# unknownue/puflow

Measured on AMD Instinct MI355X. Metric: patches/sec x4 2048->8192 (PU1K discrete, eval), higher is better.
Workload: dtype f32 (split-fp16 MFMA products, fp32 accumulate); 1 GPU; BASELINE configs[1]: PU1K discrete x4 inference, 32 x 2048-pt patches per GPU (fp32-parity mode); patches_per_gpu=32, total_batch=32, npoint=2048

## Files before the change

### puflow_amd/csrc/knn.hip

```cpp
#include <hip/hip_runtime.h>
#include "pf_api_internal.h"
#include "pf_wave.h"
#include <type_traits>

#ifndef PF_KNN5
#define PF_KNN5 1
#endif
#ifndef PF_KNN5_NWMAX
#define PF_KNN5_NWMAX 16
#endif
#ifndef PF_KNN5_MIN_M
#define PF_KNN5_MIN_M 256
#endif
#ifndef PF_KNN5_MIN_WGS
#define PF_KNN5_MIN_WGS 64
#endif
typedef float f4 __attribute__((ext_vector_type(4)));

namespace {

__device__ __forceinline__ float sqdist(float qx, float qy, float qz, float rx, float ry, float rz) {
#pragma clang fp contract(off)
    const float dx = __fsub_rn(qx, rx), dy = __fsub_rn(qy, ry), dz = __fsub_rn(qz, rz);
    return __fadd_rn(__fadd_rn(__fmul_rn(dx, dx), __fmul_rn(dy, dy)), __fmul_rn(dz, dz));
}

__device__ __forceinline__ int knn_opaque(int v) { asm("" : "+v"(v)); return v; }

template <int K>
__device__ __forceinline__ void topk_insert(float (&bd)[K], int (&bi)[K], float d, int j) {
#pragma unroll
    for (int i = K - 1; i >= 1; --i) {
        const bool ltl = d < bd[i - 1], lti = d < bd[i];
        bi[i] = ltl ? knn_opaque(bi[i - 1]) : (lti ? j : knn_opaque(bi[i]));
        bd[i] = ltl ? bd[i - 1] : (lti ? d : bd[i]);
    }
    if (d < bd[0]) { bd[0] = d; bi[0] = j; }
}

template <int K, int T>
__device__ __forceinline__ void topk_insert_head(float (&bd)[K], int (&bi)[K], float d, int j) {
    constexpr int TOP = T < K - 1 ? T : K - 1;
#pragma unroll
    for (int i = TOP; i >= 1; --i) {
        const bool ltl = d < bd[i - 1], lti = d < bd[i];
        bi[i] = ltl ? knn_opaque(bi[i - 1]) : (lti ? j : knn_opaque(bi[i]));
        bd[i] = ltl ? bd[i - 1] : (lti ? d : bd[i]);
    }
    if (d < bd[0]) { bd[0] = d; bi[0] = j; }
}

template <int I, int N, class F>
__device__ __forceinline__ void pf_static_for_knn(F&& f) {
    if constexpr (I < N) {
        f(std::integral_constant<int, I>{});
        pf_static_for_knn<I + 1, N>(f);
    }
}

template <int K>
__device__ __forceinline__ void exact_scan(float qx, float qy, float qz, const float* __restrict__ r, int M,
                                           float (&bd)[K], int (&bi)[K]) {
#pragma unroll
    for (int i = 0; i < K; ++i) { bd[i] = __builtin_inff(); bi[i] = -1; }
    for (int j = 0; j < M; ++j) {
        const float d = sqdist(qx, qy, qz, r[j * 3 + 0], r[j * 3 + 1], r[j * 3 + 2]);
        if (d < bd[K - 1]) topk_insert<K>(bd, bi, d, j);
    }
}

template <int K>
__device__ __forceinline__ void store_topk(const float (&bd)[K], const int (&bi)[K], size_t row, int* __restrict__ idx_out,
                                           float* __restrict__ dist_out) {
    if (idx_out) {
        int* o = idx_out + row * K;
#pragma unroll
        for (int i = 0; i < K; ++i) o[i] = bi[i];
    }
    if (dist_out) {
        float* od = dist_out + row * K;
#pragma unroll
        for (int i = 0; i < K; ++i) od[i] = bd[i];
    }
}

template <int K>
__global__ __launch_bounds__(64) void knn_kernel(const float* __restrict__ p1, const float* __restrict__ p2,
                                                 int N, int M, int* __restrict__ idx_out,
                                                 float* __restrict__ dist_out) {
    const int b = blockIdx.y;
    const int n = blockIdx.x * 64 + threadIdx.x;
    const bool live = n < N;
    const float* q = p1 + ((size_t)b * N + (live ? n : N - 1)) * 3;
    const float qx = q[0], qy = q[1], qz = q[2];
    float bd[K];
    int bi[K];
    exact_scan<K>(qx, qy, qz, p2 + (size_t)b * M * 3, M, bd, bi);
    if (live) store_topk<K>(bd, bi, (size_t)b * N + n, idx_out, dist_out);
}

__device__ __forceinline__ void sort16(float (&v)[16]) {
#pragma unroll
    for (int k = 2; k <= 16; k <<= 1)
#pragma unroll
        for (int j = k >> 1; j > 0; j >>= 1)
#pragma unroll
            for (int i = 0; i < 16; ++i) {
                const int l = i ^ j;
                if (l > i) {
                    const float a = v[i], c = v[l];
                    const bool up = (i & k) == 0;
                    v[i] = up ? fminf(a, c) : fmaxf(a, c);
                    v[l] = up ? fmaxf(a, c) : fminf(a, c);
                }
            }
}

constexpr int KNN2_T = 256;
constexpr int KNN2_CAP = 64;

__device__ __forceinline__ float bcast(float v, int srclane) {
    return __builtin_bit_cast(float, __builtin_amdgcn_readlane(__builtin_bit_cast(int, v), srclane));
}

template <int K>
__global__ __launch_bounds__(KNN2_T) void knn2_kernel(const float* __restrict__ p1, const float* __restrict__ p2,
                                                      int N, int M, int* __restrict__ idx_out,
                                                      float* __restrict__ dist_out) {
    static_assert(K <= 16, "threshold selection uses two 16-element sorted halves");
    __shared__ unsigned short lst[KNN2_CAP][KNN2_T];
    const int b = blockIdx.y, tid = threadIdx.x, lane = tid & 63;
    const int n = blockIdx.x * KNN2_T + tid;
    const bool live = n < N;
    const float* q = p1 + ((size_t)b * N + (live ? n : N - 1)) * 3;
    const float qx = q[0], qy = q[1], qz = q[2];
    const float* __restrict__ r = p2 + (size_t)b * M * 3;

    auto load_ref = [&](int j0, float& cx, float& cy, float& cz) {
        const int j = j0 + lane;
        const bool in = j < M;
        const int jc = in ? j : M - 1;
        cx = in ? r[jc * 3 + 0] : __builtin_inff();
        cy = r[jc * 3 + 1];
        cz = r[jc * 3 + 2];
    };

    float gm[32];
#pragma unroll
    for (int g = 0; g < 32; ++g) gm[g] = __builtin_inff();
    {
        float cx, cy, cz;
        load_ref(0, cx, cy, cz);
        for (int j0 = 0; j0 < M; j0 += 64) {
            float nx = cx, ny = cy, nz = cz;
            if (j0 + 64 < M) load_ref(j0 + 64, nx, ny, nz);
#pragma unroll
            for (int c = 0; c < 64; ++c)
                gm[c & 31] = fminf(gm[c & 31], sqdist(qx, qy, qz, bcast(cx, c), bcast(cy, c), bcast(cz, c)));
            cx = nx; cy = ny; cz = nz;
        }
    }
    float tau;
    {
        float ha[16], hb[16];
#pragma unroll
        for (int g = 0; g < 16; ++g) { ha[g] = gm[g]; hb[g] = gm[16 + g]; }
        sort16(ha);
        sort16(hb);
        tau = fminf(ha[0], hb[K - 1]);
#pragma unroll
        for (int i = 1; i < K; ++i) tau = fmaxf(tau, fminf(ha[i], hb[K - 1 - i]));
    }

    int cnt = 0;
    {
        float cx, cy, cz;
        load_ref(0, cx, cy, cz);
        for (int j0 = 0; j0 < M; j0 += 64) {
            float nx = cx, ny = cy, nz = cz;
            if (j0 + 64 < M) load_ref(j0 + 64, nx, ny, nz);
#pragma unroll
            for (int c = 0; c < 64; ++c) {
                const float d = sqdist(qx, qy, qz, bcast(cx, c), bcast(cy, c), bcast(cz, c));
                if (d <= tau) {
                    if (cnt < KNN2_CAP) lst[cnt][tid] = (unsigned short)(j0 + c);
                    ++cnt;
                }
            }
            cx = nx; cy = ny; cz = nz;
        }
    }

    float bd[K];
    int bi[K];
    if (__any(cnt > KNN2_CAP)) {
        exact_scan<K>(qx, qy, qz, r, M, bd, bi);
    } else {
#pragma unroll
        for (int i = 0; i < K; ++i) { bd[i] = __builtin_inff(); bi[i] = -1; }
        for (int s = 0; __any(s < cnt); ++s) {
            if (s < cnt) {
                const int j = lst[s][tid];
                const float d = sqdist(qx, qy, qz, r[j * 3 + 0], r[j * 3 + 1], r[j * 3 + 2]);
                topk_insert<K>(bd, bi, d, j);
            }
        }
    }
    if (live) store_topk<K>(bd, bi, (size_t)b * N + n, idx_out, dist_out);
}

#ifndef PF_KNN4_U
#define PF_KNN4_U 32
#endif
constexpr int KNN4_U = PF_KNN4_U;

template <int K, int KNN4_W>
__global__ __launch_bounds__(KNN4_W * 64) void knn4_kernel(const float* __restrict__ p1, const float* __restrict__ p2,
                                                           int N, int M, int* __restrict__ idx_out,
                                                           float* __restrict__ dist_out) {
    static_assert(K <= 16, "threshold selection uses two 16-element sorted halves");
    constexpr int KNN4_G = 32 / KNN4_W;
    constexpr int KNN4_CAP = 32;
    __shared__ float gms[32][64];
    __shared__ unsigned short lst[KNN4_W][KNN4_CAP][64];
    __shared__ int cnts[KNN4_W][64];
    const int b = blockIdx.y, lane = threadIdx.x & 63;
    const int wave = __builtin_amdgcn_readfirstlane(threadIdx.x >> 6);
    const int n = blockIdx.x * 64 + lane;
    const bool live = n < N;
    const float* q = p1 + ((size_t)b * N + (live ? n : N - 1)) * 3;
    const float qx = q[0], qy = q[1], qz = q[2];
    const float* __restrict__ r = p2 + (size_t)b * M * 3;
    auto fdist = [&](int j) {
        const float* rr = r + (size_t)j * 3;
        const float dx = qx - rr[0], dy = qy - rr[1], dz = qz - rr[2];
        return fmaf(dz, dz, fmaf(dy, dy, dx * dx));
    };
    const int mq = ((M + KNN4_W * 64 - 1) / (KNN4_W * 64)) * 64;
    const int jb = wave * mq, je = min(jb + mq, M);
    const int jfull = jb + ((je - jb) > 0 ? ((je - jb) / KNN4_U) * KNN4_U : 0);

    {
        float gm[KNN4_G];
#pragma unroll
        for (int g = 0; g < KNN4_G; ++g) gm[g] = __builtin_inff();
        for (int j0 = jb; j0 < jfull; j0 += KNN4_U) {
#pragma unroll
            for (int c = 0; c < KNN4_U; ++c) gm[c % KNN4_G] = fminf(gm[c % KNN4_G], fdist(j0 + c));
        }
        for (int j0 = jfull; j0 < je; j0 += KNN4_G) {
#pragma unroll
            for (int g = 0; g < KNN4_G; ++g)
                if (j0 + g < je) gm[g] = fminf(gm[g], fdist(j0 + g));
        }
#pragma unroll
        for (int g = 0; g < KNN4_G; ++g) gms[wave * KNN4_G + g][lane] = gm[g];
    }
    __syncthreads();
    float tau;
    {
        float ha[16], hb[16];
#pragma unroll
        for (int g = 0; g < 16; ++g) { ha[g] = gms[g][lane]; hb[g] = gms[16 + g][lane]; }
        sort16(ha);
        sort16(hb);
        tau = fminf(ha[0], hb[K - 1]);
#pragma unroll
        for (int i = 1; i < K; ++i) tau = fmaxf(tau, fminf(ha[i], hb[K - 1 - i]));
        tau = fmaf(tau, 1.9073486328125e-6f, tau) + 1e-37f;
    }

#if defined(PF_KNN_ABL) && PF_KNN_ABL == 2
    if (wave == 0 && live) idx_out[((size_t)b * N + n) * K] = __float_as_int(tau);
    return;
#endif
    int cnt = 0;
    auto take = [&](float d, int j) {
        if (d <= tau) {
            if (cnt < KNN4_CAP) lst[wave][cnt][lane] = (unsigned short)j;
            ++cnt;
        }
    };
    for (int j0 = jb; j0 < jfull; j0 += KNN4_U) {
        float dd[KNN4_U];
#pragma unroll
        for (int c = 0; c < KNN4_U; ++c) dd[c] = fdist(j0 + c);
#pragma unroll
        for (int c = 0; c < KNN4_U; c += 4) {
            if (fminf(fminf(dd[c], dd[c + 1]), fminf(dd[c + 2], dd[c + 3])) <= tau) {
                take(dd[c], j0 + c); take(dd[c + 1], j0 + c + 1); take(dd[c + 2], j0 + c + 2); take(dd[c + 3], j0 + c + 3);
            }
        }
    }
    for (int j = jfull; j < je; ++j) take(fdist(j), j);
    cnts[wave][lane] = cnt;
#if defined(PF_KNN_ABL) && PF_KNN_ABL == 1
    __syncthreads();
    if (wave == 0 && live) idx_out[((size_t)b * N + n) * K] = cnt;
    return;
#endif
    if constexpr (KNN4_W == 4) {
        static_assert(KNN4_CAP * 2 >= K * 4, "a wave's list region is reused for its K sorted distances");
        __shared__ unsigned short sidx[4][K][64];
        float (*sdst)[64] = reinterpret_cast<float (*)[64]>(&lst[wave][0][0]);
        {
            float bd[K];
            int bi[K];
#pragma unroll
            for (int i = 0; i < K; ++i) { bd[i] = __builtin_inff(); bi[i] = 0xffff; }
            const int cme = cnt < KNN4_CAP ? cnt : KNN4_CAP;
            int j = cme > 0 ? (int)lst[wave][0][lane] : 0;
            float rx = r[j * 3 + 0], ry = r[j * 3 + 1], rz = r[j * 3 + 2];
            for (int t = 0; __any(t < cme); ++t) {
                const int jn = t + 1 < cme ? (int)lst[wave][t + 1][lane] : 0;
                const float nx = r[jn * 3 + 0], ny = r[jn * 3 + 1], nz = r[jn * 3 + 2];
                if (t < cme) topk_insert<K>(bd, bi, sqdist(qx, qy, qz, rx, ry, rz), j);
                j = jn; rx = nx; ry = ny; rz = nz;
            }
#pragma unroll
            for (int i = 0; i < K; ++i) { sdst[i][lane] = bd[i]; sidx[wave][i][lane] = (unsigned short)bi[i]; }
        }
        __syncthreads();
        if (wave != 0) return;
        float bd[K];
        int bi[K];
        if (__any(cnts[0][lane] > KNN4_CAP || cnts[1][lane] > KNN4_CAP || cnts[2][lane] > KNN4_CAP || cnts[3][lane] > KNN4_CAP)) {
            exact_scan<K>(qx, qy, qz, r, M, bd, bi);
        } else {
            float hd[4];
            int hi[4], hp[4];
#pragma unroll
            for (int w = 0; w < 4; ++w) {
                hd[w] = reinterpret_cast<const float (*)[64]>(&lst[w][0][0])[0][lane];
                hi[w] = sidx[w][0][lane];
                hp[w] = 1;
            }
#pragma unroll
            for (int i = 0; i < K; ++i) {
                int wm = 0;
                float dm = hd[0];
#pragma unroll
                for (int w = 1; w < 4; ++w)
                    if (hd[w] < dm) { dm = hd[w]; wm = w; }
                int im = hi[0];
#pragma unroll
                for (int w = 1; w < 4; ++w) im = wm == w ? hi[w] : im;
                bd[i] = dm; bi[i] = im;
                int pm = hp[0];
#pragma unroll
                for (int w = 1; w < 4; ++w) pm = wm == w ? hp[w] : pm;
                const int pc = pm < K ? pm : K - 1;
                const float nd = pm < K ? reinterpret_cast<const float (*)[64]>(&lst[wm][0][0])[pc][lane] : __builtin_inff();
                const int ni = sidx[wm][pc][lane];
#pragma unroll
                for (int w = 0; w < 4; ++w) {
                    const bool m = wm == w;
                    hd[w] = m ? nd : hd[w]; hi[w] = m ? ni : hi[w]; hp[w] = m ? pm + 1 : hp[w];
                }
            }
        }
        if (live) store_topk<K>(bd, bi, (size_t)b * N + n, idx_out, dist_out);
        return;
    }
    __syncthreads();
    bool over = false;
    int ctot = 0;
#pragma unroll
    for (int w = 0; w < KNN4_W; ++w) { over |= cnts[w][lane] > KNN4_CAP; ctot += cnts[w][lane]; }
    if (__any(over || ctot > 64)) {
        if (wave != 0) return;
        float bd[K];
        int bi[K];
        exact_scan<K>(qx, qy, qz, r, M, bd, bi);
        if (live) store_topk<K>(bd, bi, (size_t)b * N + n, idx_out, dist_out);
        return;
    }
    constexpr int QPW = 64 / KNN4_W;
    int jq[QPW], cq[QPW];
    float dq[QPW];
#pragma unroll
    for (int t = 0; t < QPW; ++t) {
        const int ql = wave * QPW + t;
        cq[t] = __builtin_amdgcn_readlane(ctot, ql);
        int j0 = 0x7fffffff, acc = 0;
#pragma unroll
        for (int w = 0; w < KNN4_W; ++w) {
            const int cw = cnts[w][ql];
            const int s0 = lane - acc;
            if (s0 >= 0 && s0 < cw) j0 = lst[w][s0][ql];
            acc += cw;
        }
        jq[t] = j0;
    }
#pragma unroll
    for (int t = 0; t < QPW; ++t) {
        const int ql = wave * QPW + t;
        const float ax = __builtin_bit_cast(float, __builtin_amdgcn_readlane(__builtin_bit_cast(int, qx), ql));
        const float ay = __builtin_bit_cast(float, __builtin_amdgcn_readlane(__builtin_bit_cast(int, qy), ql));
        const float az = __builtin_bit_cast(float, __builtin_amdgcn_readlane(__builtin_bit_cast(int, qz), ql));
        const int jj = lane < cq[t] ? jq[t] : 0;
        const float d = sqdist(ax, ay, az, r[(size_t)jj * 3 + 0], r[(size_t)jj * 3 + 1], r[(size_t)jj * 3 + 2]);
        dq[t] = lane < cq[t] ? d : __builtin_inff();
    }
#pragma unroll
    for (int t = 0; t < QPW; ++t) {
        const int ql = wave * QPW + t;
        const int nq = blockIdx.x * 64 + ql;
        if (nq >= N) break;
        const int C = cq[t];
        const float d0 = dq[t];
        const int j0 = jq[t];
        const size_t row = (size_t)b * N + nq;
        int r0 = 0;
        for (int c = 0; c < C; ++c) {
            const float dc = __builtin_bit_cast(float, __builtin_amdgcn_readlane(__builtin_bit_cast(int, d0), c));
            const int jc = __builtin_amdgcn_readlane(j0, c);
            r0 += (dc < d0 || (dc == d0 && jc < j0)) ? 1 : 0;
        }
        if (lane < C && r0 < K) { idx_out[row * K + r0] = j0; if (dist_out) dist_out[row * K + r0] = d0; }
    }
}

constexpr int KNN5_CAP = 32;
constexpr int KNN5_WB = 6144;
template <int K, int NW>
__global__ __launch_bounds__(NW * 64) void knn5_kernel(const float* __restrict__ p1, const float* __restrict__ p2, int N, int M,
                                                       int Mpad, int* __restrict__ idx_out, float* __restrict__ dist_out) {
    static_assert(K <= 16, "threshold selection uses two 16-element sorted halves");
    extern __shared__ float4 k5lds[];
    __shared__ float rmx[NW];
    const int b = blockIdx.y, lane = threadIdx.x & 63, wave = threadIdx.x >> 6;
    const int col = lane & 15, g = lane >> 4;
    const int n = (blockIdx.x * NW + wave) * 16 + col;
    const bool live = n < N;
    const float* __restrict__ r = p2 + (size_t)b * M * 3;
    float4* tab = k5lds;
    unsigned char* wsm = reinterpret_cast<unsigned char*>(k5lds + Mpad) + wave * KNN5_WB;
    float (*gms)[64] = reinterpret_cast<float (*)[64]>(wsm);
    unsigned short (*lst)[64] = reinterpret_cast<unsigned short (*)[64]>(wsm + 2048);
    float rm = 0.f;
    for (int j = threadIdx.x; j < Mpad; j += NW * 64) {
        float4 e = make_float4(0.f, 0.f, 0.f, __builtin_inff());
        if (j < M) {
            const float x = r[j * 3 + 0], y = r[j * 3 + 1], z = r[j * 3 + 2];
            const float R = fmaf(z, z, fmaf(y, y, x * x));
            e = make_float4(-2.f * x, -2.f * y, -2.f * z, R);
            rm = fmaxf(rm, R);
        }
        tab[j] = e;
    }
    rm = pf_xor_max<1, 32>(rm);
    if (lane == 0) rmx[wave] = rm;
    __syncthreads();
    float Rmax = rmx[0];
#pragma unroll
    for (int w = 1; w < NW; ++w) Rmax = fmaxf(Rmax, rmx[w]);
#if defined(PF_KNN_ABL) && PF_KNN_ABL == 3
    if (live && g == 0) idx_out[((size_t)b * N + n) * K] = __float_as_int(Rmax);
    return;
#endif
    if ((blockIdx.x * NW + wave) * 16 >= N) return;
    const float* qp = p1 + ((size_t)b * N + (live ? n : N - 1)) * 3;
    const float qx = qp[0], qy = qp[1], qz = qp[2];
    const float bq = g == 0 ? qx : (g == 1 ? qy : (g == 2 ? qz : 1.f));
    const float* tabf = reinterpret_cast<const float*>(tab) + col * 4 + g;
    const int nch = Mpad / 16;
    auto filtc = [&](int c, f4 acc) { return __builtin_amdgcn_mfma_f32_16x16x4f32(tabf[c * 64], bq, acc, 0, 0, 0); };
    auto filt = [&](int c) {
        const f4 z4 = {0.f, 0.f, 0.f, 0.f};
        return filtc(c, z4);
    };
    {
        float gm[8];
#pragma unroll
        for (int i = 0; i < 8; ++i) gm[i] = __builtin_inff();
        for (int c0 = 0; c0 < nch; c0 += 8) {
            f4 d[8];
#pragma unroll
            for (int u = 0; u < 8; ++u) d[u] = filt(c0 + u);
            __builtin_amdgcn_sched_barrier(0);
#pragma unroll
            for (int u = 0; u < 8; u += 4)
#pragma unroll
                for (int v = 0; v < 2; ++v)
#pragma unroll
                    for (int i = 0; i < 4; ++i)
                        gm[v * 4 + i] = __builtin_fminf(gm[v * 4 + i], __builtin_fminf(d[u + v][i], d[u + v + 2][i]));
        }
#pragma unroll
        for (int i = 0; i < 8; ++i) gms[i][lane] = gm[i];
    }
    __builtin_amdgcn_wave_barrier();
    float tau;
    {
        float ha[16], hb[16];
#pragma unroll
        for (int i = 0; i < 8; ++i) {
            ha[i] = gms[i][col]; ha[8 + i] = gms[i][col + 16];
            hb[i] = gms[i][col + 32]; hb[8 + i] = gms[i][col + 48];
        }
        if constexpr (K == 1) {
            tau = fminf(ha[0], hb[0]);
#pragma unroll
            for (int i = 1; i < 16; ++i) tau = fminf(tau, fminf(ha[i], hb[i]));
        } else {
            sort16(ha);
            sort16(hb);
            tau = fminf(ha[0], hb[K - 1]);
#pragma unroll
            for (int i = 1; i < K; ++i) tau = fmaxf(tau, fminf(ha[i], hb[K - 1 - i]));
        }
        const float s = __builtin_sqrtf(Rmax) + __builtin_sqrtf(fmaf(qz, qz, fmaf(qy, qy, qx * qx)));
        tau = fmaf(3.814697265625e-6f, s * s, tau) + 4e-37f;
    }
#if defined(PF_KNN_ABL) && PF_KNN_ABL == 2
    if (live && g == 0) idx_out[((size_t)b * N + n) * K] = __float_as_int(tau);
    return;
#endif
    int cnt = 0;
    const f4 ntau = {-tau, -tau, -tau, -tau};
    for (int c0 = 0; c0 < nch; c0 += 8) {
        f4 d[8];
#pragma unroll
        for (int u = 0; u < 8; ++u) d[u] = filtc(c0 + u, ntau);
        __builtin_amdgcn_sched_barrier(0);
        unsigned m0 = 0, m1 = 0, m2 = 0, m3 = 0;
#pragma unroll
        for (int s = 0; s < 8; ++s) {
            const int u = s >> 2, i = s & 3;
            asm("v_alignbit_b32 %0, %0, %4, 31\n\tv_alignbit_b32 %1, %1, %5, 31\n\t"
                "v_alignbit_b32 %2, %2, %6, 31\n\tv_alignbit_b32 %3, %3, %7, 31"
                : "+v"(m0), "+v"(m1), "+v"(m2), "+v"(m3)
                : "v"(d[u][i]), "v"(d[2 + u][i]), "v"(d[4 + u][i]), "v"(d[6 + u][i]));
        }
        unsigned mask = (m0 << 24) | (m1 << 16) | (m2 << 8) | m3;
        auto pop = [&]() {
            if (mask != 0) {
                const int p = __clz((int)mask);
                mask &= ~(0x80000000u >> p);
                lst[cnt & (KNN5_CAP - 1)][lane] = (unsigned short)((c0 + (p >> 2)) * 16 + 4 * g + (p & 3));
                ++cnt;
            }
        };
#if defined(PF_KNN_ABL) && PF_KNN_ABL == 6
        cnt += __popc(mask);
#else
        pop();
        pop();
        while (__any(mask != 0)) pop();
#endif
    }
#if defined(PF_KNN_ABL) && (PF_KNN_ABL == 1 || PF_KNN_ABL == 6)
    if (live && g == 0) idx_out[((size_t)b * N + n) * K] = cnt;
    return;
#endif
    float bd[K];
    int bi[K];
    {
#pragma unroll
        for (int i = 0; i < K; ++i) { bd[i] = __builtin_inff(); bi[i] = 0xffff; }
        const int cme = cnt < KNN5_CAP ? cnt : KNN5_CAP;
        auto dist_of = [&](int t) {
            int j = lst[t][lane];
            j = j < Mpad ? j : 0;
            const float4 e = tab[j];
            return t < cme ? sqdist(qx, qy, qz, -0.5f * e.x, -0.5f * e.y, -0.5f * e.z) : __builtin_inff();
        };
        pf_static_for_knn<0, (K + 3) / 4>([&](auto gc) {
            constexpr int G4 = decltype(gc)::value;
            if (G4 == 0 || __any(cme > 4 * G4)) {
                float dd[4];
#pragma unroll
                for (int k = 0; k < 4; ++k) dd[k] = dist_of(4 * G4 + k);
                pf_static_for_knn<0, 4>([&](auto kc) {
                    constexpr int T = 4 * G4 + decltype(kc)::value;
                    if (T < K) topk_insert_head<K, T>(bd, bi, dd[T - 4 * G4], (int)lst[T][lane]);
                });
            }
        });
        for (int t = K; __any(t < cme); ++t) {
            if (t < cme) {
                const int j = lst[t][lane];
                const float4 e = tab[j];
                topk_insert<K>(bd, bi, sqdist(qx, qy, qz, -0.5f * e.x, -0.5f * e.y, -0.5f * e.z), j);
            }
        }
    }
#if defined(PF_KNN_ABL) && PF_KNN_ABL == 5
    if (live && g == 0) idx_out[((size_t)b * N + n) * K] = bi[0] + bi[K - 1];
    return;
#endif
    __builtin_amdgcn_wave_barrier();
    float (*sd)[64] = reinterpret_cast<float (*)[64]>(wsm);
    unsigned short (*si)[64] = reinterpret_cast<unsigned short (*)[64]>(wsm + 4096);
    static_assert(K * 64 * 4 <= 4096 && 4096 + K * 64 * 2 <= KNN5_WB, "per-wave scratch holds the sorted lists");
#pragma unroll
    for (int i = 0; i < K; ++i) { sd[i][lane] = bd[i]; si[i][lane] = (unsigned short)bi[i]; }
    __builtin_amdgcn_wave_barrier();
    const int ctot = pf_xor_sum<16, 32>(cnt), cmax = pf_xor_max<16, 32>(cnt);
#if defined(PF_KNN_ABL) && PF_KNN_ABL == 4
    if (false) {
#else
    if (__any(cmax > KNN5_CAP || ctot < K)) {
#endif
        exact_scan<K>(qx, qy, qz, r, M, bd, bi);
        if (live && g == 0) store_topk<K>(bd, bi, (size_t)b * N + n, idx_out, dist_out);
        return;
    }
    if (g != 0) return;
    float hd[4];
    int hi[4], hp[4];
#pragma unroll
    for (int w = 0; w < 4; ++w) { hd[w] = sd[0][col + 16 * w]; hi[w] = si[0][col + 16 * w]; hp[w] = 1; }
#pragma unroll
    for (int i = 0; i < K; ++i) {
        int wm = 0;
        float dm = hd[0];
        int im = hi[0];
#pragma unroll
        for (int w = 1; w < 4; ++w)
            if (hd[w] < dm || (hd[w] == dm && hi[w] < im)) { dm = hd[w]; im = hi[w]; wm = w; }
        bd[i] = dm; bi[i] = im;
        int pm = hp[0];
#pragma unroll
        for (int w = 1; w < 4; ++w) pm = wm == w ? hp[w] : pm;
        const int pc = pm < K ? pm : K - 1;
        const float nd = pm < K ? sd[pc][col + 16 * wm] : __builtin_inff();
        const int ni = pm < K ? (int)si[pc][col + 16 * wm] : 0xffff;
#pragma unroll
        for (int w = 0; w < 4; ++w) {
            const bool m = wm == w;
            hd[w] = m ? nd : hd[w]; hi[w] = m ? ni : hi[w]; hp[w] = m ? pm + 1 : hp[w];
        }
    }
    if (live) store_topk<K>(bd, bi, (size_t)b * N + n, idx_out, dist_out);
}

__device__ __forceinline__ void nn1_body(const float* __restrict__ q1, const float* __restrict__ r, int N, int M, int n,
                                         float* __restrict__ dout, int* __restrict__ iout) {
    const bool live = n < N;
    const float* q = q1 + (size_t)(live ? n : N - 1) * 3;
    const float qx = q[0], qy = q[1], qz = q[2];
    float best = __builtin_inff(), thr = __builtin_inff();
    int besti = 0;
    auto visit = [&](int j) {
        const float* rr = r + (size_t)j * 3;
        const float d = sqdist(qx, qy, qz, rr[0], rr[1], rr[2]);
        const bool lt = d < best;
        best = lt ? d : best;
        besti = lt ? j : besti;
    };
    auto filt = [&](int j) {
        const float* rr = r + (size_t)j * 3;
        const float dx = qx - rr[0], dy = qy - rr[1], dz = qz - rr[2];
        return fmaf(dz, dz, fmaf(dy, dy, dx * dx));
    };
    const int mfull = (M / 32) * 32;
    for (int j0 = 0; j0 < mfull; j0 += 32) {
        float f[32];
#pragma unroll
        for (int c = 0; c < 32; ++c) f[c] = filt(j0 + c);
#pragma unroll
        for (int c = 0; c < 32; c += 4) {
            if (fminf(fminf(f[c], f[c + 1]), fminf(f[c + 2], f[c + 3])) < thr) {
                visit(j0 + c); visit(j0 + c + 1); visit(j0 + c + 2); visit(j0 + c + 3);
                thr = fmaf(best, 9.5367431640625e-7f, best) + 1e-37f;
            }
        }
    }
    for (int j = mfull; j < M; ++j) visit(j);
    if (live) {
        dout[n] = best;
        if (iout) iout[n] = besti;
    }
}

__global__ __launch_bounds__(256) void nn1_kernel(const float* __restrict__ p1, const float* __restrict__ p2,
                                                  int N, int M, float* __restrict__ dist_out,
                                                  int* __restrict__ idx_out) {
    const int b = blockIdx.y;
    nn1_body(p1 + (size_t)b * N * 3, p2 + (size_t)b * M * 3, N, M, blockIdx.x * 256 + threadIdx.x, dist_out + (size_t)b * N,
             idx_out ? idx_out + (size_t)b * N : nullptr);
}

constexpr int NN1_RAGGED_MAXB = 64;
struct Nn1RaggedTab {
    int xoff[NN1_RAGGED_MAXB], n[NN1_RAGGED_MAXB];
    int yoff[NN1_RAGGED_MAXB], m[NN1_RAGGED_MAXB];
    int t0[NN1_RAGGED_MAXB + 1];
};
__global__ __launch_bounds__(256) void nn1_ragged_kernel(const float* __restrict__ p1, const float* __restrict__ p2,
                                                         const Nn1RaggedTab t, int nc, float* __restrict__ dist_out,
                                                         int* __restrict__ idx_out) {
    int c = 0;
    while (c + 1 < nc && (int)blockIdx.x >= t.t0[c + 1]) ++c;
    nn1_body(p1 + (size_t)t.xoff[c] * 3, p2 + (size_t)t.yoff[c] * 3, t.n[c], t.m[c], ((int)blockIdx.x - t.t0[c]) * 256 + threadIdx.x,
             dist_out + t.xoff[c], idx_out ? idx_out + t.xoff[c] : nullptr);
}


template <int K>
static void launch_knn5(const float* p1, const float* p2, int B, int N, int M, int* idx_out, float* dist_out, hipStream_t s) {
    const int Mpad = (M + 127) / 128 * 128;
    int ncu = 256, dev = 0;
    if (hipGetDevice(&dev) == hipSuccess) (void)hipDeviceGetAttribute(&ncu, hipDeviceAttributeMultiprocessorCount, dev);
    int NW = PF_KNN5_NWMAX;
    while (NW > 4 && ((long long)B * ((N + 16 * NW - 1) / (16 * NW)) < ncu || (size_t)Mpad * 16 + (size_t)NW * KNN5_WB > 150 * 1024)) NW >>= 1;
    const size_t lds = (size_t)Mpad * 16 + (size_t)NW * KNN5_WB;
    const dim3 g5((N + 16 * NW - 1) / (16 * NW), B);
#define PF_KNN5_LAUNCH(W)                                                                                                 \
    do { allow_lds(knn5_kernel<K, W>, lds);                                            \
         hipLaunchKernelGGL((knn5_kernel<K, W>), g5, dim3(W * 64), lds, s, p1, p2, N, M, Mpad, idx_out, dist_out); } while (0)
    if (NW == 16) PF_KNN5_LAUNCH(16); else if (NW == 8) PF_KNN5_LAUNCH(8); else PF_KNN5_LAUNCH(4);
#undef PF_KNN5_LAUNCH
}

static bool use_knn5(int B, int N, int M) {
#if PF_KNN5
    const long long wgs = (long long)((N + 63) / 64) * B;
    return wgs >= PF_KNN5_MIN_WGS && (M >= 1024 || (M >= PF_KNN5_MIN_M && wgs <= 1024)) && M <= 4096;
#else
    (void)B; (void)N; (void)M;
    return false;
#endif
}

}

extern "C" int pf_knn(const float* p1, const float* p2, int B, int N, int M, int K, int* idx_out,
                      float* dist_out, void* stream) {
    if (!p1 || !p2 || !idx_out) return PF_ERR_NULL;
    if (B <= 0 || N <= 0 || M <= 0 || K <= 0 || K > M || B > 65535) return PF_ERR_SHAPE;
    hipStream_t s = (hipStream_t)stream;
    if (K <= 16 && M >= (PF_KNN5_MIN_M < 1024 ? PF_KNN5_MIN_M : 1024) && M <= 65536) {
        const dim3 g4((N + 63) / 64, B);
        const long long wgs = (long long)g4.x * B;
        if (use_knn5(B, N, M) && (K == 4 || K == 8 || K == 16)) {
            switch (K) {
                case 4:  launch_knn5<4>(p1, p2, B, N, M, idx_out, dist_out, s); break;
                case 8:  launch_knn5<8>(p1, p2, B, N, M, idx_out, dist_out, s); break;
                default: launch_knn5<16>(p1, p2, B, N, M, idx_out, dist_out, s); break;
            }
            return pf_last_launch_status();
        }
        if (M >= 1024) {
        const int W = wgs >= 1024 ? 4 : (wgs >= 384 ? 8 : 16);
#define PF_KNN4_LAUNCH(KK)                                                                                              \
        if (W == 4) hipLaunchKernelGGL((knn4_kernel<KK, 4>), g4, dim3(256), 0, s, p1, p2, N, M, idx_out, dist_out);         \
        else if (W == 8) hipLaunchKernelGGL((knn4_kernel<KK, 8>), g4, dim3(512), 0, s, p1, p2, N, M, idx_out, dist_out);    \
        else hipLaunchKernelGGL((knn4_kernel<KK, 16>), g4, dim3(1024), 0, s, p1, p2, N, M, idx_out, dist_out)
        switch (K) {
            case 4:  PF_KNN4_LAUNCH(4); break;
            case 8:  PF_KNN4_LAUNCH(8); break;
            case 16: PF_KNN4_LAUNCH(16); break;
            default: return PF_ERR_UNSUPPORTED;
        }
#undef PF_KNN4_LAUNCH
        return pf_last_launch_status();
        }
    }
    if (K <= 16 && M >= 256 && M <= 65536) {
        dim3 g2((N + KNN2_T - 1) / KNN2_T, B), b2(KNN2_T);
        switch (K) {
            case 4:  hipLaunchKernelGGL(knn2_kernel<4>, g2, b2, 0, s, p1, p2, N, M, idx_out, dist_out); break;
            case 8:  hipLaunchKernelGGL(knn2_kernel<8>, g2, b2, 0, s, p1, p2, N, M, idx_out, dist_out); break;
            case 16: hipLaunchKernelGGL(knn2_kernel<16>, g2, b2, 0, s, p1, p2, N, M, idx_out, dist_out); break;
            default: return PF_ERR_UNSUPPORTED;
        }
        return pf_last_launch_status();
    }
    dim3 grid((N + 63) / 64, B), block(64);
    switch (K) {
        case 8:  hipLaunchKernelGGL(knn_kernel<8>, grid, block, 0, s, p1, p2, N, M, idx_out, dist_out); break;
        case 16: hipLaunchKernelGGL(knn_kernel<16>, grid, block, 0, s, p1, p2, N, M, idx_out, dist_out); break;
        case 4:  hipLaunchKernelGGL(knn_kernel<4>, grid, block, 0, s, p1, p2, N, M, idx_out, dist_out); break;
        case 32: hipLaunchKernelGGL(knn_kernel<32>, grid, block, 0, s, p1, p2, N, M, idx_out, dist_out); break;
        default: return PF_ERR_UNSUPPORTED;
    }
    return pf_last_launch_status();
}

extern "C" int pf_nn1(const float* p1, const float* p2, int B, int N, int M, float* dist_out, int* idx_out,
                      void* stream) {
    if (!p1 || !p2 || !dist_out) return PF_ERR_NULL;
    if (B <= 0 || N <= 0 || M <= 0 || B > 65535) return PF_ERR_SHAPE;
    if (use_knn5(B, N, M)) {
        launch_knn5<1>(p1, p2, B, N, M, idx_out, dist_out, (hipStream_t)stream);
        return pf_last_launch_status();
    }
    hipLaunchKernelGGL(nn1_kernel, dim3((N + 255) / 256, B), dim3(256), 0, (hipStream_t)stream, p1, p2, N, M, dist_out,
                       idx_out);
    return pf_last_launch_status();
}

extern "C" int pf_nn1_ragged(const float* p1, const float* p2, const int* n, const int* m, int B, float* dist_out, int* idx_out,
                             void* stream) {
    if (!p1 || !p2 || !n || !m || !dist_out) return PF_ERR_NULL;
    if (B <= 0) return PF_ERR_SHAPE;
    long long nt = 0, mt = 0;
    for (int i = 0; i < B; ++i) {
        if (n[i] <= 0 || m[i] <= 0) return PF_ERR_SHAPE;
        nt += n[i]; mt += m[i];
    }
    if (nt * 3 > 0x7fffffffll || mt * 3 > 0x7fffffffll) return PF_ERR_SHAPE;
    hipStream_t s = (hipStream_t)stream;
    Nn1RaggedTab t;
    int nc = 0;
    auto launch = [&]() {
        if (!nc) return;
        hipLaunchKernelGGL(nn1_ragged_kernel, dim3(t.t0[nc]), dim3(256), 0, s, p1, p2, t, nc, dist_out, idx_out);
        nc = 0;
    };
    long long xoff = 0, yoff = 0;
    for (int i = 0; i < B; ++i) {
        if (use_knn5(1, n[i], m[i])) {
            launch_knn5<1>(p1 + xoff * 3, p2 + yoff * 3, 1, n[i], m[i], idx_out ? idx_out + xoff : nullptr, dist_out + xoff, s);
        } else {
            if (nc == 0) t.t0[0] = 0;
            t.xoff[nc] = (int)xoff; t.n[nc] = n[i]; t.yoff[nc] = (int)yoff; t.m[nc] = m[i];
            t.t0[nc + 1] = t.t0[nc] + (n[i] + 255) / 256;
            if (++nc == NN1_RAGGED_MAXB) launch();
        }
        xoff += n[i]; yoff += m[i];
    }
    launch();
    return pf_last_launch_status();
}
```

Before: 27780 patches/s.

## Switch KNN5 distance filter from fp32 MFMA to split-fp16 MFMA

```diff
diff --git a/puflow_amd/csrc/knn.hip b/puflow_amd/csrc/knn.hip
--- a/puflow_amd/csrc/knn.hip
+++ b/puflow_amd/csrc/knn.hip
@@ -1,6 +1,6 @@
 #include <hip/hip_runtime.h>
 #include "pf_api_internal.h"
-#include "pf_wave.h"
+#include "pf_mfma.h"
 #include <type_traits>
 
 #ifndef PF_KNN5
@@ -15,7 +15,6 @@
 #ifndef PF_KNN5_MIN_WGS
 #define PF_KNN5_MIN_WGS 64
 #endif
-typedef float f4 __attribute__((ext_vector_type(4)));
 
 namespace {
 
@@ -423,6 +422,16 @@
 
 constexpr int KNN5_CAP = 32;
 constexpr int KNN5_WB = 6144;
+constexpr float KNN5_PAD = 60000.f;
+constexpr float KNN5_QMAX = 64.f;
+
+struct Knn5Split { _Float16 h, l; };
+__device__ __forceinline__ Knn5Split knn5_split(float v) {
+    const _Float16 h = (_Float16)v;
+    return Knn5Split{h, (_Float16)(v - (float)h)};
+}
+__device__ __forceinline__ unsigned knn5_pk(_Float16 a, _Float16 b) { return __builtin_bit_cast(unsigned, (h2){a, b}); }
+
 template <int K, int NW>
 __global__ __launch_bounds__(NW * 64) void knn5_kernel(const float* __restrict__ p1, const float* __restrict__ p2, int N, int M,
                                                        int Mpad, int* __restrict__ idx_out, float* __restrict__ dist_out) {
@@ -438,16 +447,38 @@
     unsigned char* wsm = reinterpret_cast<unsigned char*>(k5lds + Mpad) + wave * KNN5_WB;
     float (*gms)[64] = reinterpret_cast<float (*)[64]>(wsm);
     unsigned short (*lst)[64] = reinterpret_cast<unsigned short (*)[64]>(wsm + 2048);
+    const float inf = __builtin_inff();
+    float cm = 0.f;
+    for (int j = threadIdx.x; j < Mpad; j += NW * 64) {
+        float4 e = make_float4(inf, 0.f, 0.f, 0.f);
+        if (j < M) {
+            e = make_float4(r[j * 3 + 0], r[j * 3 + 1], r[j * 3 + 2], 0.f);
+            const float ax = fabsf(e.x), ay = fabsf(e.y), az = fabsf(e.z);
+            if (ax < inf && ay < inf && az < inf) cm = fmaxf(cm, fmaxf(ax, fmaxf(ay, az)));
+        }
+        tab[j] = e;
+    }
+    cm = pf_xor_max<1, 32>(cm);
+    if (lane == 0) *reinterpret_cast<float*>(wsm) = cm;
+    __syncthreads();
+    float cmax = 0.f;
+#pragma unroll
+    for (int w = 0; w < NW; ++w) cmax = fmaxf(cmax, *reinterpret_cast<const float*>(reinterpret_cast<const unsigned char*>(k5lds + Mpad) + w * KNN5_WB));
+    const int es = min(4 - ((int)(__float_as_uint(cmax) >> 23) - 127), 62);
+    const float s = __uint_as_float((unsigned)(127 + es) << 23);
     float rm = 0.f;
+    u4* tabh = reinterpret_cast<u4*>(tab);
     for (int j = threadIdx.x; j < Mpad; j += NW * 64) {
-        float4 e = make_float4(0.f, 0.f, 0.f, __builtin_inff());
-        if (j < M) {
-            const float x = r[j * 3 + 0], y = r[j * 3 + 1], z = r[j * 3 + 2];
+        const float4 e = tab[j];
+        u4 t = {0u, knn5_pk((_Float16)0.f, (_Float16)KNN5_PAD), 0u, 0u};
+        if (fabsf(e.x) < inf && fabsf(e.y) < inf && fabsf(e.z) < inf) {
+            const float x = s * e.x, y = s * e.y, z = s * e.z;
             const float R = fmaf(z, z, fmaf(y, y, x * x));
-            e = make_float4(-2.f * x, -2.f * y, -2.f * z, R);
             rm = fmaxf(rm, R);
-        }
-        tab[j] = e;
+            const Knn5Split X = knn5_split(-2.f * x), Y = knn5_split(-2.f * y), Z = knn5_split(-2.f * z), RR = knn5_split(R);
+            t = (u4){knn5_pk(X.h, Y.h), knn5_pk(Z.h, RR.h), knn5_pk(X.l, Y.l), knn5_pk(Z.l, RR.l)};
+        }
+        tabh[j] = t;
     }
     rm = pf_xor_max<1, 32>(rm);
     if (lane == 0) rmx[wave] = rm;
@@ -462,10 +493,19 @@
     if ((blockIdx.x * NW + wave) * 16 >= N) return;
     const float* qp = p1 + ((size_t)b * N + (live ? n : N - 1)) * 3;
     const float qx = qp[0], qy = qp[1], qz = qp[2];
-    const float bq = g == 0 ? qx : (g == 1 ? qy : (g == 2 ? qz : 1.f));
-    const float* tabf = reinterpret_cast<const float*>(tab) + col * 4 + g;
+    float sx = s * qx, sy = s * qy, sz = s * qz;
+    const bool qbad = !(fabsf(sx) <= KNN5_QMAX && fabsf(sy) <= KNN5_QMAX && fabsf(sz) <= KNN5_QMAX);
+    if (qbad) sx = sy = sz = 0.f;
+    h8 bq;
+    {
+        const Knn5Split X = knn5_split(sx), Y = knn5_split(sy), Z = knn5_split(sz);
+        const unsigned h0 = knn5_pk(X.h, Y.h), h1 = knn5_pk(Z.h, (_Float16)1.f);
+        const u4 r0 = {h0, h1, h0, h1}, r1 = {knn5_pk(X.l, Y.l), knn5_pk(Z.l, (_Float16)0.f), 0u, 0u}, z = {0u, 0u, 0u, 0u};
+        bq = __builtin_bit_cast(h8, g == 0 ? r0 : (g == 1 ? r1 : z));
+    }
+    const u4* tabq = tabh + col;
     const int nch = Mpad / 16;
-    auto filtc = [&](int c, f4 acc) { return __builtin_amdgcn_mfma_f32_16x16x4f32(tabf[c * 64], bq, acc, 0, 0, 0); };
+    auto filtc = [&](int c, f4 acc) { return pf_mfma_f16(__builtin_bit_cast(h8, tabq[c * 16]), bq, acc); };
     auto filt = [&](int c) {
         const f4 z4 = {0.f, 0.f, 0.f, 0.f};
         return filtc(c, z4);
@@ -479,13 +519,17 @@
 #pragma unroll
             for (int u = 0; u < 8; ++u) d[u] = filt(c0 + u);
             __builtin_amdgcn_sched_barrier(0);
-#pragma unroll
-            for (int u = 0; u < 8; u += 4)
-#pragma unroll
-                for (int v = 0; v < 2; ++v)
-#pragma unroll
-                    for (int i = 0; i < 4; ++i)
-                        gm[v * 4 + i] = __builtin_fminf(gm[v * 4 + i], __builtin_fminf(d[u + v][i], d[u + v + 2][i]));
+#define PF_KNN5_MIN3(U, PRE)                                                                                                   \
+            asm(PRE "v_min3_f32 %0, %0, %8, %16\n\tv_min3_f32 %1, %1, %9, %17\n\tv_min3_f32 %2, %2, %10, %18\n\t"             \
+                    "v_min3_f32 %3, %3, %11, %19\n\tv_min3_f32 %4, %4, %12, %20\n\tv_min3_f32 %5, %5, %13, %21\n\t"           \
+                    "v_min3_f32 %6, %6, %14, %22\n\tv_min3_f32 %7, %7, %15, %23"                                              \
+                : "+v"(gm[0]), "+v"(gm[1]), "+v"(gm[2]), "+v"(gm[3]), "+v"(gm[4]), "+v"(gm[5]), "+v"(gm[6]), "+v"(gm[7])       \
+                : "v"(d[U][0]), "v"(d[U][1]), "v"(d[U][2]), "v"(d[U][3]), "v"(d[U + 1][0]), "v"(d[U + 1][1]), "v"(d[U + 1][2]),  \
+                  "v"(d[U + 1][3]), "v"(d[U + 2][0]), "v"(d[U + 2][1]), "v"(d[U + 2][2]), "v"(d[U + 2][3]), "v"(d[U + 3][0]),    \
+                  "v"(d[U + 3][1]), "v"(d[U + 3][2]), "v"(d[U + 3][3]))
+            PF_KNN5_MIN3(0, "");
+            PF_KNN5_MIN3(4, "s_nop 3\n\t");
+#undef PF_KNN5_MIN3
         }
 #pragma unroll
         for (int i = 0; i < 8; ++i) gms[i][lane] = gm[i];
@@ -510,8 +554,8 @@
 #pragma unroll
             for (int i = 1; i < K; ++i) tau = fmaxf(tau, fminf(ha[i], hb[K - 1 - i]));
         }
-        const float s = __builtin_sqrtf(Rmax) + __builtin_sqrtf(fmaf(qz, qz, fmaf(qy, qy, qx * qx)));
-        tau = fmaf(3.814697265625e-6f, s * s, tau) + 4e-37f;
+        const float S = __builtin_sqrtf(Rmax) + __builtin_sqrtf(fmaf(sz, sz, fmaf(sy, sy, sx * sx)));
+        tau += 1.7881393432617188e-7f * fmaf(S, fmaf(40.f, S, 2.f), 2.f);
     }
 #if defined(PF_KNN_ABL) && PF_KNN_ABL == 2
     if (live && g == 0) idx_out[((size_t)b * N + n) * K] = __float_as_int(tau);
@@ -562,9 +606,9 @@
         const int cme = cnt < KNN5_CAP ? cnt : KNN5_CAP;
         auto dist_of = [&](int t) {
             int j = lst[t][lane];
-            j = j < Mpad ? j : 0;
-            const float4 e = tab[j];
-            return t < cme ? sqdist(qx, qy, qz, -0.5f * e.x, -0.5f * e.y, -0.5f * e.z) : __builtin_inff();
+            j = j < M ? j : 0;
+            const float* rr = r + j * 3;
+            return t < cme ? sqdist(qx, qy, qz, rr[0], rr[1], rr[2]) : __builtin_inff();
         };
         pf_static_for_knn<0, (K + 3) / 4>([&](auto gc) {
             constexpr int G4 = decltype(gc)::value;
@@ -581,8 +625,8 @@
         for (int t = K; __any(t < cme); ++t) {
             if (t < cme) {
                 const int j = lst[t][lane];
-                const float4 e = tab[j];
-                topk_insert<K>(bd, bi, sqdist(qx, qy, qz, -0.5f * e.x, -0.5f * e.y, -0.5f * e.z), j);
+                const float* rr = r + j * 3;
+                topk_insert<K>(bd, bi, sqdist(qx, qy, qz, rr[0], rr[1], rr[2]), j);
             }
         }
     }
@@ -597,11 +641,11 @@
 #pragma unroll
     for (int i = 0; i < K; ++i) { sd[i][lane] = bd[i]; si[i][lane] = (unsigned short)bi[i]; }
     __builtin_amdgcn_wave_barrier();
-    const int ctot = pf_xor_sum<16, 32>(cnt), cmax = pf_xor_max<16, 32>(cnt);
+    const int ctot = pf_xor_sum<16, 32>(cnt), cmx = pf_xor_max<16, 32>(cnt);
 #if defined(PF_KNN_ABL) && PF_KNN_ABL == 4
     if (false) {
 #else
-    if (__any(cmax > KNN5_CAP || ctot < K)) {
+    if (__any(cmx > KNN5_CAP || ctot < K || qbad)) {
 #endif
         exact_scan<K>(qx, qy, qz, r, M, bd, bi);
         if (live && g == 0) store_topk<K>(bd, bi, (size_t)b * N + n, idx_out, dist_out);
```

After: 28010 patches/s (median of 6 runs). Within noise of the previous version (+0.8%).
